# ml-jku/LaM-SLidE

Measured on AMD Instinct MI355X. Metric: sampled trajectories/sec (50-step ODE) + decoded-coord L2 vs ref, MD17, higher is better.
Workload: dtype bf16; 1 GPU; md17_bench; tail=False, ln_fuse=True, T=30, L=256, C=32, D=512, H=16, depth=4, sampler=ODE, state_updates=50, batch_per_gpu=32, global_batch=32, parallelism=batch-shard x1, 1 gather to rank 0 per step, noise_elem_stride_per_rank=7864320, kernels=general, trajectories_per_pass=32

## Files before the change

### lam_slide_amd/csrc/k_lin1.hip.h

```cpp
#pragma once
#include <type_traits>

#include "common.hip.h"

struct Lin1Args {
    const u16 *W;
    const u16 *X;
    const float *bias;
    const float4 *rope_q, *rope_k;
    u16 *qkv;
    u16 *z;
    int F, N, HHD, M;
    int pos_div, pos_mod;
    unsigned div_magic, mod_magic;
    float inv_hd, q_premul;
    int nt;
    int wpt;
    int planes;
    int npad;
    const float2 *ln_stat;
    const float *ln_shift, *ln_scale;
    int ln_mod_stride, ln_tpt;
    unsigned ln_tpt_magic;
};

#ifndef LIN1_B2
#define LIN1_B2 1
#endif
#ifndef LIN1_B2_KMAX
#define LIN1_B2_KMAX 256
#endif

template <int HDP, int K, int NW = 8>
struct Lin1Cfg {
    static_assert(K % 128 == 0 && K <= 512, "hidden sizes 128 / 256 / 384 / 512");
    static constexpr int KS = K / 16;
    static constexpr int ROWB = 2 * K;
    static constexpr int PITCH = ROWB + 16;
    static constexpr int BLK = 32 * PITCH;
    static constexpr int NS = (LIN1_B2 && K <= LIN1_B2_KMAX) ? 4 : 3;
    static constexpr int RING = NS * BLK;
    static_assert(NW == 8 || NW == 4, "two waves per SIMD (256-token tiles) or one (128-token tiles)");
    static constexpr int TT = 32 * NW;
    static constexpr int STAGE = NW * 4096;
    static constexpr int LPR = ROWB / 16;
    static constexpr int PPW = 32 / NW;
    static constexpr size_t lds_bytes(int F) { return (size_t)RING + STAGE + (size_t)F * 4; }
    static constexpr int LN_SLOTS = K <= 256 ? 3 : 2;
    static constexpr size_t lds_bytes_lnf(int F) { return lds_bytes(F) + (size_t)LN_SLOTS * 2 * K * 4; }
};

enum { LIN1_QK = 0, LIN1_V = 1, LIN1_MLP = 2 };

#ifndef LIN1_XLOAD
#define LIN1_XLOAD 1
#endif
#ifndef LIN1_PD
#define LIN1_PD 3
#endif

__device__ __forceinline__ float lin1_gelu(float x) {
    const float ax = fabsf(x);
    const float h = __builtin_amdgcn_exp2f(LSL_GELU_Q(ax));
    float relu;
    asm("v_max_f32 %0, 0, %1" : "=v"(relu) : "v"(x));
    return fmaf(-ax, h, relu);
}

template <int HDP, int K, int NW = 8, bool LNF = false>
__global__ void __launch_bounds__(NW * 64, NW / 4) k_linear1_ts(Lin1Args g) {
    using C = Lin1Cfg<HDP, K, NW>;
    constexpr int KS = C::KS, BLK = C::BLK, PPW = C::PPW, ROWB = C::ROWB;
    constexpr int NCO = HDP == 32 ? 8 : 4;
    extern __shared__ __attribute__((aligned(16))) char smem[];

    const int tid = threadIdx.x, lane = tid & 63;
    const int wave = __builtin_amdgcn_readfirstlane(tid >> 6);
    const int r = lane & 31, hf = lane >> 5;
    char *const stage = smem + C::RING + wave * 4096;
    float *const bias_lds = reinterpret_cast<float *>(smem + C::RING + C::STAGE);

    const int NB = g.F >> 5;
    const int ntile = (g.N + C::TT - 1) / C::TT;
    const long U = (long)ntile * NB;
    long i0, i1;
    if (g.wpt > 0) {
        const int tile = blockIdx.x / g.wpt, part = blockIdx.x - tile * g.wpt;
        i0 = (long)tile * NB + ((NB * part / g.wpt) & ~1);
        i1 = (long)tile * NB + (part + 1 == g.wpt ? NB : ((NB * (part + 1) / g.wpt) & ~1));
    } else {
        i0 = (U * blockIdx.x / gridDim.x) & ~1L;
        i1 = blockIdx.x + 1 == gridDim.x ? U : ((U * (blockIdx.x + 1) / gridDim.x) & ~1L);
    }
    if (i0 >= i1) return;

    for (int i = tid * 4; i < g.F; i += NW * 64 * 4) *reinterpret_cast<float4 *>(bias_lds + i) = *reinterpret_cast<const float4 *>(g.bias + i);

    const unsigned lds0 = (unsigned)(size_t)(LDS_PTR(char))(smem);
    const unsigned lane_src = lane * 16;
    const char *const w_rows = reinterpret_cast<const char *>(g.W) + (size_t)(PPW * wave) * ROWB;
    auto issue_piece = [&](const char *src, unsigned dst, auto ic) __attribute__((always_inline)) {
        constexpr int I = decltype(ic)::value & 3;
        if (decltype(ic)::value >= 4) {
            src += 4 * ROWB;
            dst += 4 * C::PITCH;
        }
        const unsigned ls = lane_src;
        if (C::LPR == 64 || lane < C::LPR) {
            if (I == 0 || decltype(ic)::value >= 4)
                asm volatile("s_add_u32 m0, %2, %3\n\ts_nop 4\n\tglobal_load_lds_dwordx4 %0, %1 offset:%4" ::"v"(ls), "s"(src), "s"(dst), "n"(16 * I), "n"(ROWB * I) : "memory", "scc");
            else
                asm volatile("s_add_u32 m0, %2, %3\n\ts_nop 0\n\tglobal_load_lds_dwordx4 %0, %1 offset:%4" ::"v"(ls), "s"(src), "s"(dst), "n"(16 * I), "n"(ROWB * I) : "memory", "scc");
        }
    };
    auto req_src = [&](int blk) __attribute__((always_inline)) { return w_rows + (size_t)blk * (32 * ROWB); };
    auto req_dst = [&](int slot) __attribute__((always_inline)) { return lds0 + slot * BLK + PPW * wave * C::PITCH; };
    auto issue = [&](int blk, int slot) __attribute__((always_inline)) {
        const char *src = req_src(blk);
        const unsigned dst = req_dst(slot);
        issue_piece(src, dst, std::integral_constant<int, 0>());
        issue_piece(src, dst, std::integral_constant<int, 1>());
        issue_piece(src, dst, std::integral_constant<int, 2>());
        issue_piece(src, dst, std::integral_constant<int, 3>());
        if (PPW == 8) {
            issue_piece(src, dst, std::integral_constant<int, 4>());
            issue_piece(src, dst, std::integral_constant<int, 5>());
            issue_piece(src, dst, std::integral_constant<int, 6>());
            issue_piece(src, dst, std::integral_constant<int, 7>());
        }
    };
    const int aoff = r * C::PITCH + 16 * hf;

    bf16x8 xreg[KS];
    float4 co[NCO];
    f32x16 acc0, acc1;
    int slot_c = 0;
    int dma_blk, dma_slot;
    int n_wave = 0;
    float post = 1.0f;

    auto advance = [&](int &b) __attribute__((always_inline)) { b = b + 1 == NB ? 0 : b + 1; };
    auto next_slot = [&](int s) __attribute__((always_inline)) { return s == C::NS - 1 ? 0 : s + 1; };

    {
        int b = (int)(i0 - (i0 / NB) * NB);
        issue(b, 0);
        advance(b);
        issue(b, 1);
        advance(b);
        dma_blk = b;
        dma_slot = 2;
    }

    auto init_acc = [&](f32x16 &a, int blk) __attribute__((always_inline)) {
#pragma unroll
        for (int q4 = 0; q4 < 4; ++q4) {
            const float4 b = *reinterpret_cast<const float4 *>(bias_lds + blk * 32 + 8 * q4 + 4 * hf);
            a[4 * q4] = b.x; a[4 * q4 + 1] = b.y; a[4 * q4 + 2] = b.z; a[4 * q4 + 3] = b.w;
        }
    };
    constexpr bool B2 = LIN1_B2 != 0 && K <= LIN1_B2_KMAX;
    auto step_head = [&](auto flushed_c) __attribute__((always_inline)) {
        if (B2) {
            if (decltype(flushed_c)::value) wait_vmcnt<PPW>();
            else wait_vmcnt<0>();
        } else {
            if (decltype(flushed_c)::value) wait_vmcnt<2 * PPW>();
            else wait_vmcnt<PPW>();
        }
        __builtin_amdgcn_s_barrier();
        asm volatile("" ::: "memory");
    };
    const unsigned wr0 = (unsigned)(size_t)(LDS_PTR(char))(stage) + r * 128 + 8 * hf + ((r & 7) << 4);
    const unsigned rd0 = (unsigned)(size_t)(LDS_PTR(char))(stage) + (lane >> 3) * 128 + (((lane & 7) ^ ((lane >> 3) & 7)) << 4);
    const char *row_q = nullptr, *row_z = nullptr;
    const bool planes = g.planes != 0;
    constexpr unsigned PROW = 2u * HDP, CPH = HDP / 8;
    const unsigned plane_bytes = PROW * (unsigned)g.npad;
    const unsigned stride_q = planes ? PROW : 2u * 3 * g.HHD, stride_z = 2u * (g.HHD + g.M);
    const unsigned blk_q = planes ? (32 / HDP) * plane_bytes : 64u;
    const unsigned voff_q = planes ? ((lane & 7) / CPH) * plane_bytes + (lane >> 3) * PROW + 16 * ((lane & 7) % CPH) : (lane >> 3) * stride_q + 16 * (lane & 7);
    const unsigned voff_z = (lane >> 3) * stride_z + 16 * (lane & 7);
    const int slab_z = 3 * (g.HHD >> 5);
    const char *fl_base = nullptr;
    unsigned fl_stride8 = 0, fl_voff = 0;
    auto flush_setup = [&](int b_even) __attribute__((always_inline)) {
        const bool to_qkv = b_even < slab_z;
        fl_base = to_qkv ? row_q : row_z;
        fl_stride8 = 8 * (to_qkv ? stride_q : stride_z);
        fl_voff = to_qkv ? voff_q + blk_q * (unsigned)b_even : voff_z + 64u * (unsigned)b_even;
    };
    auto flush_read = [&](int half, u32x4 (&pk)[2]) __attribute__((always_inline)) {
#pragma unroll
        for (int i = 0; i < 2; ++i) pk[i] = *reinterpret_cast<const LDS_PTR(u32x4)>(rd0 + 1024 * (2 * half + i));
    };
    auto flush_store = [&](int half, const u32x4 (&pk)[2]) __attribute__((always_inline)) {
        asm volatile("s_nop 4\n\tglobal_store_dwordx4 %0, %1, %2 nt\n\ts_nop 1" ::"v"(fl_voff + (2 * half) * fl_stride8), "v"(pk[0]), "s"(fl_base) : "memory");
        asm volatile("global_store_dwordx4 %0, %1, %2 nt\n\ts_nop 1" ::"v"(fl_voff + (2 * half + 1) * fl_stride8), "v"(pk[1]), "s"(fl_base) : "memory");
    };
    auto flush_store_visible = [&](int half, const u32x4 (&pk)[2]) __attribute__((always_inline)) {
#pragma unroll
        for (int i = 0; i < 2; ++i)
            __builtin_nontemporal_store(pk[i], reinterpret_cast<u32x4 *>(const_cast<char *>(fl_base) + (size_t)(fl_voff + (2 * half + i) * fl_stride8)));
    };
    auto put_group = [&](int ii, int q, float v0, float v1, float v2, float v3) __attribute__((always_inline)) {
        const u32x2 pk = {pack2(v0, v1), pack2(v2, v3)};
        *reinterpret_cast<LDS_PTR(u32x2)>(wr0 ^ (unsigned)(64 * ii + 16 * q)) = pk;
    };
    auto epi_slice = [&](auto sec_c, int s, const f32x16 &a, int ii, float &c0, float &c1) __attribute__((always_inline)) {
        constexpr int SEC = decltype(sec_c)::value;
        if constexpr (SEC == LIN1_QK && HDP == 32) {
            if (s == 0) c0 = 0.0f;
            if (s < 2) {
#pragma unroll
                for (int e = 0; e < 8; ++e) c0 = fmaf(a[8 * s + e], a[8 * s + e], c0);
            }
            if (s == 1) c0 = rsqrtf(fmaf(half_pair_sum(c0), g.inv_hd, 1e-6f)) * post;
            if (s >= 2 && s < 6) {
                const int q = s - 2;
                float o[4];
#pragma unroll
                for (int kk = 0; kk < 2; ++kk) {
                    const int k = 2 * q + kk;
                    const float x0 = a[2 * k], x1 = a[2 * k + 1];
                    o[2 * kk] = c0 * fmaf(co[k].x, x0, -co[k].y * x1);
                    o[2 * kk + 1] = c0 * fmaf(co[k].z, x0, co[k].w * x1);
                }
                put_group(ii, q, o[0], o[1], o[2], o[3]);
            }
        } else if constexpr (SEC == LIN1_QK) {
            if (s == 0) {
                c0 = 0.0f;
#pragma unroll
                for (int e = 0; e < 8; ++e) c0 = fmaf(a[e], a[e], c0);
            }
            if (s == 1) {
                c1 = 0.0f;
#pragma unroll
                for (int e = 0; e < 8; ++e) c1 = fmaf(a[8 + e], a[8 + e], c1);
                c0 = rsqrtf(fmaf(half_pair_sum(c0), g.inv_hd, 1e-6f)) * post;
                c1 = rsqrtf(fmaf(half_pair_sum(c1), g.inv_hd, 1e-6f)) * post;
            }
            if (s >= 2 && s < 6) {
                const int q = s - 2;
                const float rr = q < 2 ? c0 : c1;
                float o[4];
#pragma unroll
                for (int kk = 0; kk < 2; ++kk) {
                    const int k = 2 * q + kk;
                    const float x0 = a[2 * k], x1 = a[2 * k + 1];
                    const float4 cf = co[k & (NCO - 1)];
                    o[2 * kk] = rr * fmaf(cf.x, x0, -cf.y * x1);
                    o[2 * kk + 1] = rr * fmaf(cf.z, x0, cf.w * x1);
                }
                put_group(ii, q, o[0], o[1], o[2], o[3]);
            }
        } else if constexpr (SEC == LIN1_MLP) {
            const float g0 = lin1_gelu(a[2 * s]), g1 = lin1_gelu(a[2 * s + 1]);
            if (s & 1) put_group(ii, s >> 1, c0, c1, g0, g1);
            else { c0 = g0; c1 = g1; }
        } else {
            if (s < 4) put_group(ii, s, a[4 * s], a[4 * s + 1], a[4 * s + 2], a[4 * s + 3]);
        }
    };
    auto step = [&](auto sec_c, auto par_c, auto mfma_c, auto epi_c, auto side) __attribute__((always_inline)) {
        constexpr int PAR = decltype(par_c)::value;
        constexpr bool DO_MFMA = decltype(mfma_c)::value != 0, DO_EPI = decltype(epi_c)::value != 0;
        constexpr int MPS = KS / 8, PD = LIN1_PD, MH = (MPS + 1) / 2;
        f32x16 &ac = PAR ? acc0 : acc1;
        const f32x16 &ae = PAR ? acc1 : acc0;
        const char *sb = smem + slot_c * BLK + aoff;
        bf16x8 fr[PD];
        float c0 = 0.0f, c1 = 0.0f;
        if (DO_MFMA) {
#pragma unroll
            for (int ks = 0; ks < PD; ++ks) fr[ks] = as_bf16x8(*reinterpret_cast<const u32x4 *>(sb + 32 * ks));
        }
        side(std::integral_constant<int, -1>());
#define LIN1_SIDE(S) if (s == S) side(std::integral_constant<int, S>());
#pragma unroll
        for (int s = 0; s < 8; ++s) {
#pragma unroll
            for (int m = 0; m < MPS; ++m) {
                if (m == MH) { LIN1_SIDE(0) LIN1_SIDE(1) LIN1_SIDE(2) LIN1_SIDE(3) LIN1_SIDE(4) LIN1_SIDE(5) LIN1_SIDE(6) LIN1_SIDE(7) }
                if (DO_MFMA) {
                    const int ks = s * MPS + m;
                    ac = mfma32(fr[ks % PD], xreg[ks], ac);
                    if (ks + PD < KS) fr[ks % PD] = as_bf16x8(*reinterpret_cast<const u32x4 *>(sb + 32 * (ks + PD)));
                }
            }
            if (MH == MPS) { LIN1_SIDE(0) LIN1_SIDE(1) LIN1_SIDE(2) LIN1_SIDE(3) LIN1_SIDE(4) LIN1_SIDE(5) LIN1_SIDE(6) LIN1_SIDE(7) }
            if (DO_EPI) epi_slice(sec_c, s, ae, PAR, c0, c1);
            __builtin_amdgcn_sched_barrier(0);
        }
#undef LIN1_SIDE
        if (decltype(mfma_c)::value != 0) slot_c = next_slot(slot_c);
    };
    std::integral_constant<int, 0> I0;
    std::integral_constant<int, 1> I1;
    auto no_side = [](auto) __attribute__((always_inline)) {};
    auto fused = [&](auto sec_c, auto par_c, auto flush_c, auto prev_c, int e) __attribute__((always_inline)) {
        constexpr int PAR = decltype(par_c)::value;
        constexpr bool FLUSH = decltype(flush_c)::value != 0;
        if (!B2 || PAR == 1) step_head(prev_c);
        u32x4 pk[2];
        if (FLUSH) flush_setup(e - 2);
        const char *src = req_src(dma_blk);
        const unsigned dst = req_dst(dma_slot);
        int blk2 = dma_blk;
        advance(blk2);
        const char *src2 = req_src(blk2);
        const unsigned dst2 = req_dst(next_slot(dma_slot));
        init_acc(PAR ? acc0 : acc1, e + 1);
        step(sec_c, par_c, I1, I1, [&](auto sl) __attribute__((always_inline)) {
            constexpr int SL = decltype(sl)::value;
            if (FLUSH) {
                if (SL == -1) flush_read(0, pk);
                if (SL == 0) {
                    flush_store(0, pk);
                    flush_read(1, pk);
                }
                if (SL == 1) flush_store(1, pk);
            }
            constexpr int PS = PPW / 4;
            if (!B2) {
                if (SL >= 2 && SL < 6) {
                    issue_piece(src, dst, std::integral_constant<int, (SL >= 2 && SL < 6) ? PS * (SL - 2) : 0>());
                    if (PS == 2) issue_piece(src, dst, std::integral_constant<int, (SL >= 2 && SL < 6) ? PS * (SL - 2) + 1 : 0>());
                }
            } else if (PAR == 1) {
                if (SL >= 0 && SL < 4) {
                    issue_piece(src, dst, std::integral_constant<int, (SL >= 0 && SL < 4) ? PS * SL : 0>());
                    if (PS == 2) issue_piece(src, dst, std::integral_constant<int, (SL >= 0 && SL < 4) ? PS * SL + 1 : 0>());
                }
                if (SL >= 4 && SL < 8) {
                    issue_piece(src2, dst2, std::integral_constant<int, (SL >= 4 && SL < 8) ? PS * (SL - 4) : 0>());
                    if (PS == 2) issue_piece(src2, dst2, std::integral_constant<int, (SL >= 4 && SL < 8) ? PS * (SL - 4) + 1 : 0>());
                }
            }
        });
        if (!B2) {
            advance(dma_blk);
            dma_slot = next_slot(dma_slot);
        } else if (PAR == 1) {
            advance(dma_blk);
            advance(dma_blk);
            dma_slot = next_slot(next_slot(dma_slot));
        }
    };
    auto run = [&](auto sec_c, int ea, int eb) __attribute__((always_inline)) {
        int e = ea;
        if (e < eb && (e & 1)) {
            fused(sec_c, I1, I0, I0, e);
            ++e;
        }
        for (; e + 1 < eb; e += 2) {
            fused(sec_c, I0, I1, I0, e);
            fused(sec_c, I1, I0, I1, e + 1);
        }
        if (e < eb) fused(sec_c, I0, I1, I0, e);
    };
    auto load_co = [&](const float4 *tab, unsigned pos) __attribute__((always_inline)) {
        const float4 *t = tab + (size_t)pos * (HDP / 2) + 2 * hf;
#pragma unroll
        for (int k = 0; k < NCO; ++k) co[k] = t[4 * (k >> 1) + (k & 1)];
    };
    std::integral_constant<int, LIN1_QK> SQK;
    std::integral_constant<int, LIN1_V> SV;
    std::integral_constant<int, LIN1_MLP> SMLP;

    constexpr bool XLINES = LIN1_XLOAD != 0 && (K <= 384 || LIN1_XLOAD >= 2);
    auto load_x = [&](int nw) __attribute__((always_inline)) {
        if (!XLINES) {
            const u16 *xr = g.X + (size_t)(nw + r) * K + 8 * hf;
#pragma unroll
            for (int ks = 0; ks < KS; ++ks) xreg[ks] = as_bf16x8(*reinterpret_cast<const u32x4 *>(xr + 16 * ks));
        } else {
            const u16 *xr = g.X + (size_t)(nw + (lane >> 3)) * K + 8 * (lane & 7);
#pragma unroll
            for (int j = 0; j < KS / 4; ++j)
#pragma unroll
                for (int q = 0; q < 4; ++q) xreg[4 * j + q] = as_bf16x8(*reinterpret_cast<const u32x4 *>(xr + (size_t)(8 * q) * K + 64 * j));
        }
    };
    auto finish_x = [&]() __attribute__((always_inline)) {
        if (!XLINES) return;
        const unsigned t0 = lane >> 3;
        const unsigned xw = (unsigned)(size_t)(LDS_PTR(char))(stage) + t0 * 128;
        const unsigned xr0 = (unsigned)(size_t)(LDS_PTR(char))(stage) + r * 128;
#pragma unroll
        for (int j = 0; j < KS / 4; ++j) {
#pragma unroll
            for (int q = 0; q < 4; ++q)
                *reinterpret_cast<LDS_PTR(u32x4)>(xw + 1024 * q + ((((lane & 7) ^ ((t0 >> 1) + 4 * q)) & 7) << 4)) = as_u32x4(xreg[4 * j + q]);
#pragma unroll
            for (int m = 0; m < 4; ++m)
                xreg[4 * j + m] = as_bf16x8(*reinterpret_cast<const LDS_PTR(u32x4)>(xr0 + ((((2 * m + hf) ^ (r >> 1)) & 7) << 4)));
        }
    };

    float *const ln_tab = bias_lds + ((g.F + 3) & ~3);
    auto traj_of = [&](unsigned n) __attribute__((always_inline)) { return g.ln_tpt_magic ? __umulhi(n, g.ln_tpt_magic) : n; };
    auto load_x_lnf = [&](int tile_, int nw) __attribute__((always_inline)) {
        typedef __attribute__((ext_vector_type(4))) float f4;
        const float *xf = reinterpret_cast<const float *>(g.X);
        const unsigned t_first = g.ln_mod_stride ? traj_of((unsigned)(tile_ * C::TT)) : 0u;
        const unsigned t_last = g.ln_mod_stride ? traj_of((unsigned)(g.N - 1)) : 0u;
        for (int i = tid * 4; i < C::LN_SLOTS * K; i += NW * 64 * 4) {
            const int slot = i / K, col = i - slot * K;
            const size_t mo = (size_t)min(t_first + (unsigned)slot, t_last) * g.ln_mod_stride + col;
            const f4 sc = *reinterpret_cast<const f4 *>(g.ln_scale + mo), sh = *reinterpret_cast<const f4 *>(g.ln_shift + mo);
            *reinterpret_cast<f4 *>(ln_tab + (size_t)slot * 2 * K + col) = f4{1.0f + sc[0], 1.0f + sc[1], 1.0f + sc[2], 1.0f + sc[3]};
            *reinterpret_cast<f4 *>(ln_tab + (size_t)slot * 2 * K + K + col) = sh;
        }
        const unsigned rowi = lane >> 3, chunk = lane & 7;
        const unsigned sbase = (unsigned)(size_t)(LDS_PTR(char))(stage);
        const unsigned xr0 = sbase + r * 128;
        const float *xr = xf + (size_t)(nw + rowi) * K + 4 * chunk;
        float2 st[4];
        const float *tb[4];
#pragma unroll
        for (int q = 0; q < 4; ++q) {
            const unsigned nn = (unsigned)min(nw + (int)rowi + 8 * q, g.N - 1);
            st[q] = g.ln_stat[nn];
            const unsigned slot = g.ln_mod_stride ? min(traj_of(nn) - t_first, (unsigned)(C::LN_SLOTS - 1)) : 0u;
            tb[q] = ln_tab + (size_t)slot * 2 * K + 4 * chunk;
        }
        __syncthreads();
#pragma unroll
        for (int p = 0; p < K / 64; ++p) {
            f4 v[2][4];
#pragma unroll
            for (int e = 0; e < 2; ++e)
#pragma unroll
                for (int q = 0; q < 4; ++q) v[e][q] = *reinterpret_cast<const f4 *>(xr + (size_t)(8 * q) * K + 64 * p + 32 * e);
#pragma unroll
            for (int q = 0; q < 4; ++q) {
                const unsigned row = rowi + 8 * q, sw = (row >> 1) & 7;
#pragma unroll
                for (int e = 0; e < 2; ++e) {
                    const f4 sc = *reinterpret_cast<const f4 *>(tb[q] + 64 * p + 32 * e), sh = *reinterpret_cast<const f4 *>(tb[q] + K + 64 * p + 32 * e);
                    f4 x = v[e][q];
#pragma unroll
                    for (int c = 0; c < 4; ++c) x[c] = fmaf(x[c], st[q].x, st[q].y) * sc[c] + sh[c];
                    const u32x2 pk = {pack2(x[0], x[1]), pack2(x[2], x[3])};
                    *reinterpret_cast<LDS_PTR(u32x2)>(sbase + row * 128 + ((((4 * e + (chunk >> 1)) ^ sw) & 7) << 4) + 8 * (chunk & 1)) = pk;
                }
            }
#pragma unroll
            for (int m = 0; m < 4; ++m)
                xreg[4 * p + m] = as_bf16x8(*reinterpret_cast<const LDS_PTR(u32x4)>(xr0 + ((((2 * m + hf) ^ (r >> 1)) & 7) << 4)));
            __builtin_amdgcn_sched_barrier(0);
        }
    };
    const int qb = g.HHD >> 5;
    int tile = (int)(i0 / NB), b0 = (int)(i0 - (long)tile * NB), left = (int)(i1 - i0);
    bool first_seg = true;
    bool co_ready = false;
    __syncthreads();
    while (left > 0) {
        const int b1 = NB - b0 < left ? NB : b0 + left;
        n_wave = tile * C::TT + wave * 32;
        row_q = reinterpret_cast<const char *>(g.qkv) + (size_t)n_wave * stride_q;
        row_z = reinterpret_cast<const char *>(g.z) + (size_t)n_wave * stride_z - 4 * (size_t)g.HHD;
        if constexpr (LNF) load_x_lnf(tile, n_wave);
        else {
            if (first_seg) load_x(n_wave);
            finish_x();
        }
        const unsigned nn = (unsigned)min(n_wave + r, g.N - 1);
        const unsigned n1 = g.div_magic ? __umulhi(nn, g.div_magic) : nn;
        const unsigned pos = g.mod_magic ? n1 - __umulhi(n1, g.mod_magic) * (unsigned)g.pos_mod : 0u;

        if (first_seg) wait_vmcnt<0>();
        else wait_vmcnt<4>();
        __builtin_amdgcn_s_barrier();
        asm volatile("" ::: "memory");
        issue(dma_blk, dma_slot);
        advance(dma_blk);
        dma_slot = next_slot(dma_slot);
        if (B2) {
            issue(dma_blk, dma_slot);
            advance(dma_blk);
            dma_slot = next_slot(dma_slot);
        }
        init_acc(acc0, b0);
        step(SV, I1, I1, I0, no_side);
        const int e_end = b1 - 1;
        if (b0 < 2 * qb) {
            if (!co_ready) load_co(b0 < qb ? g.rope_q : g.rope_k, pos);
            post = b0 < qb ? g.q_premul : 1.0f;
            fused(SQK, I0, I0, I0, b0);
        } else if (b0 < 3 * qb) {
            fused(SV, I0, I0, I0, b0);
        } else {
            fused(SMLP, I0, I0, I0, b0);
        }
        {
            const int lo = max(b0 + 1, 0), hi = min(e_end, qb);
            if (lo < hi) run(SQK, lo, hi);
        }
        {
            const int lo = max(b0 + 1, qb), hi = min(e_end, 2 * qb);
            if (lo < hi) {
                if (lo == qb) {
                    load_co(g.rope_k, pos);
                    post = 1.0f;
                }
                run(SQK, lo, hi);
            }
        }
        {
            const int lo = max(b0 + 1, 2 * qb), hi = min(e_end, 3 * qb);
            if (lo < hi) run(SV, lo, hi);
        }
        {
            const int lo = max(b0 + 1, 3 * qb), hi = min(e_end, NB);
            if (lo < hi) run(SMLP, lo, hi);
        }
        const int left_next = left - (b1 - b0);
        co_ready = false;
        if (left_next > 0) {
            asm volatile("" ::: "memory");
            const int nw = (tile + 1) * C::TT + wave * 32;
            if constexpr (!LNF) load_x(nw);
            if (b1 - 1 >= 2 * qb) {
                const unsigned nn2 = (unsigned)min(nw + r, g.N - 1);
                const unsigned m1 = g.div_magic ? __umulhi(nn2, g.div_magic) : nn2;
                load_co(g.rope_q, g.mod_magic ? m1 - __umulhi(m1, g.mod_magic) * (unsigned)g.pos_mod : 0u);
                co_ready = true;
            }
            asm volatile("" ::: "memory");
        }
        {
            const int e = b1 - 1;
            if (e < 2 * qb) {
                step(SQK, I1, I0, I1, no_side);
            } else if (e < 3 * qb) {
                step(SV, I1, I0, I1, no_side);
            } else {
                step(SMLP, I1, I0, I1, no_side);
            }
            flush_setup(e - 1);
            u32x4 pk[2];
            flush_read(0, pk);
            flush_store_visible(0, pk);
            flush_read(1, pk);
            flush_store_visible(1, pk);
        }
        left = left_next;
        tile += 1;
        b0 = 0;
        first_seg = false;
    }
    wait_vmcnt<0>();
}
```

### lam_slide_amd/csrc/k_lin2.hip.h

```cpp
#pragma once
#include <type_traits>

#include "common.hip.h"

struct Lin2Args {
    const u16 *Wp;
    const u16 *Z;
    const float *bias;
    const float *gate;
    float *h;
    int F, N;
    int mod_stride, tpt;
    unsigned tpt_magic;
    int slices, rpx;
    int gate_rows;
    float2 *stats;
    int npad;
};

#ifndef LIN2_PD
#define LIN2_PD 2
#endif

template <int N, int I = 0, class F>
__device__ __forceinline__ void static_for(F &f) {
    if constexpr (I < N) {
        f(std::integral_constant<int, I>());
        static_for<N, I + 1>(f);
    }
}

template <int K, int NCH, int NS, bool HB2>
struct Lin2Cfg {
    static_assert(K % (32 * NCH) == 0, "K / 2 splits into NCH chunks of whole 16-deep k-steps");
    static_assert(NCH >= 3 && NS >= 3, "epilogue schedule: arithmetic, stores, residual request in chunks 0, 1, 2");
    static constexpr int KH = K / 2;
    static constexpr int KSH = KH / 16;
    static constexpr int KC = KH / NCH;
    static constexpr int MPC = KC / 16;
    static constexpr int ROWB = 4 * KC;
    static constexpr int LPR = ROWB / 16;
    static_assert(LPR <= 64, "one DMA instruction per token row");
    static constexpr int PITCH = ROWB + 16;
    static constexpr int CHUNK = 32 * PITCH;
    static constexpr int RING = NS * CHUNK;
    static constexpr int EXCH = RING;
    static constexpr int HBUF = EXCH + 4 * 4096;
    static constexpr int HB_PER_WAVE = HB2 ? 8192 : 4096;
    static constexpr int BIAS = HBUF + 4 * HB_PER_WAVE;
    static constexpr int GATE = BIAS + 512;
    static constexpr size_t lds_bytes(int gate_rows) { return (size_t)GATE + (size_t)gate_rows * 512; }
    static constexpr int max_gate_rows = (163840 - GATE) / 512;
    static_assert(max_gate_rows >= 1, "LDS budget (160 KiB per workgroup)");
};

__global__ void __launch_bounds__(256) k_lin2_pack(u16 *out, const u16 *W, int F, int K) {
    const int ksh = K / 32;
    const long total = (long)(F / 32) * 2 * ksh * 64;
    for (long i = (long)blockIdx.x * 256 + threadIdx.x; i < total; i += (long)gridDim.x * 256) {
        const int lane = (int)(i & 63);
        long t = i >> 6;
        const int ks = (int)(t % ksh);
        t /= ksh;
        const int o = (int)(t & 1), fb = (int)(t >> 1);
        const u16 *src = W + (size_t)(32 * fb + (lane & 31)) * K + o * (K / 2) + 16 * ks + 8 * (lane >> 5);
        *reinterpret_cast<u32x4 *>(out + i * 8) = *reinterpret_cast<const u32x4 *>(src);
    }
}

template <int K, int NCH, int NS, bool HB2, bool LNS = false>
__global__ void __launch_bounds__(512, 2) k_linear2_ws(Lin2Args g) {
    using C = Lin2Cfg<K, NCH, NS, HB2>;
    constexpr int KSH = C::KSH, KC = C::KC, MPC = C::MPC, PITCH = C::PITCH, CHUNK = C::CHUNK, PD = LIN2_PD;
    extern __shared__ __attribute__((aligned(16))) char smem[];

    const int tid = threadIdx.x, lane = tid & 63;
    const int wave = __builtin_amdgcn_readfirstlane(tid >> 6);
    const int r = lane & 31, hf = lane >> 5;
    const int hi = wave >> 2;
    const int p = wave & 3;

    const int xcd = blockIdx.x & 7, idx = blockIdx.x >> 3;
    const int slice = idx % g.slices, range = xcd * g.rpx + idx / g.slices, ranges = 8 * g.rpx;
    const int NBLK = (g.N + 31) >> 5;
    const int blk0 = (int)((long)NBLK * range / ranges), blk1 = (int)((long)NBLK * (range + 1) / ranges);
    const int nblk = blk1 - blk0;
    if (nblk <= 0) return;
    const int f0 = slice * 128 + 32 * p;

    const unsigned lds0 = (unsigned)(size_t)(LDS_PTR(char))(smem);
    float *const bias_lds = reinterpret_cast<float *>(smem + C::BIAS);
    float *const gate_lds = reinterpret_cast<float *>(smem + C::GATE);

    bf16x8 wreg[KSH];
    {
        const u32x4 *wp = reinterpret_cast<const u32x4 *>(g.Wp) + ((size_t)((slice * 4 + p) * 2 + hi) * KSH) * 64 + lane;
#pragma unroll
        for (int ks = 0; ks < KSH; ++ks) wreg[ks] = as_bf16x8(wp[(size_t)ks * 64]);
    }
    const int n_lo = blk0 * 32, n_hi = min(blk1 * 32, g.N) - 1;
    const unsigned traj_lo = g.mod_stride ? (g.tpt_magic ? __umulhi((unsigned)n_lo, g.tpt_magic) : (unsigned)n_lo) : 0u;
    {
        const unsigned traj_hi = g.mod_stride ? (g.tpt_magic ? __umulhi((unsigned)n_hi, g.tpt_magic) : (unsigned)n_hi) : 0u;
        const int rows = min((int)(traj_hi - traj_lo) + 1, g.gate_rows);
        if (tid < 32) *reinterpret_cast<float4 *>(bias_lds + 4 * tid) = *reinterpret_cast<const float4 *>(g.bias + slice * 128 + 4 * tid);
        for (int i = tid; i < rows * 32; i += 512) {
            const int row = i >> 5, c4 = i & 31;
            *reinterpret_cast<float4 *>(gate_lds + row * 128 + 4 * c4) =
                *reinterpret_cast<const float4 *>(g.gate + (size_t)(traj_lo + row) * g.mod_stride + slice * 128 + 4 * c4);
        }
    }

    const unsigned half_lanes = C::LPR / 2;
    const unsigned voff_same = lane < half_lanes ? 16u * lane : (unsigned)K + 16u * (lane - half_lanes);
    const unsigned voff_next = lane < half_lanes ? 64u * K + 16u * lane : (unsigned)K + 16u * (lane - half_lanes);
    auto dma_row = [&](const char *src_, unsigned dst_, unsigned voff) __attribute__((always_inline)) {
        const char *src = uni_ptr(src_);
        const unsigned dst = __builtin_amdgcn_readfirstlane(dst_);
        if (C::LPR == 64 || lane < C::LPR) lds_dma16(voff, src, dst);
    };
    auto chunk_src = [&](int m, int j, unsigned &voff) __attribute__((always_inline)) {
        int mh = min(max(m - 1, 0), nblk - 1), ml = min(m, nblk - 1);
        voff = ml > mh ? voff_next : voff_same;
        return reinterpret_cast<const char *>(g.Z) + ((size_t)(blk0 + mh) * 32 + 8 * p) * (2 * K) + (size_t)j * (2 * KC);
    };

    const int boff = r * PITCH + (hi * KC + 8 * hf) * 2;
    f32x16 acc;
#pragma unroll
    for (int e = 0; e < 16; ++e) acc[e] = 0.0f;

    auto chain = [&](auto jc, int slot, bool zero_start, auto side) __attribute__((always_inline)) {
        constexpr int J = decltype(jc)::value;
        const char *sb = smem + slot * CHUNK + boff;
        bf16x8 fr[PD];
#pragma unroll
        for (int i = 0; i < PD; ++i) fr[i] = as_bf16x8(*reinterpret_cast<const u32x4 *>(sb + 32 * i));
#pragma unroll
        for (int i = 0; i < MPC; ++i) {
            if (J == 0 && i == 0 && zero_start) {
                f32x16 z;
#pragma unroll
                for (int e = 0; e < 16; ++e) z[e] = 0.0f;
                acc = mfma32(wreg[J * MPC + i], fr[i % PD], z);
            } else
                acc = mfma32(wreg[J * MPC + i], fr[i % PD], acc);
            if (i + PD < MPC) fr[i % PD] = as_bf16x8(*reinterpret_cast<const u32x4 *>(sb + 32 * (i + PD)));
            side(i);
            __builtin_amdgcn_sched_barrier(0);
        }
    };
    char *const exch = smem + C::EXCH + p * 4096;
    auto next_slot = [](int s) __attribute__((always_inline)) { return s + 1 == NS ? 0 : s + 1; };

    __builtin_amdgcn_s_waitcnt(0x0F70);
    __syncthreads();

    if (!hi) {
        int rq_m = 0, rq_j = 0, rq_slot = 0;
        auto rq_advance = [&]() __attribute__((always_inline)) {
            if (++rq_j == NCH) { rq_j = 0; ++rq_m; }
            rq_slot = next_slot(rq_slot);
        };
#pragma unroll
        for (int c = 0; c < NS - 1; ++c) {
            unsigned voff;
            const char *src = chunk_src(rq_m, rq_j, voff);
            const unsigned dst = lds0 + rq_slot * CHUNK + 8 * p * PITCH;
#pragma unroll
            for (int i = 0; i < 8; ++i) dma_row(src + (size_t)i * (2 * K), dst + i * PITCH, voff);
            rq_advance();
        }
        int slot = 0;
        for (int m = 0; m <= nblk; ++m) {
            const bool work = m < nblk;
            auto step = [&](auto jc) __attribute__((always_inline)) {
                wait_vmcnt<8 * (NS - 2)>();
                __builtin_amdgcn_s_barrier();
                asm volatile("" ::: "memory");
                unsigned voff;
                const char *src = chunk_src(rq_m, rq_j, voff);
                const unsigned dst = lds0 + rq_slot * CHUNK + 8 * p * PITCH;
                rq_advance();
                if (work) {
                    chain(jc, slot, true, [&](int i) __attribute__((always_inline)) {
                        if (i % 2 == 1 && i / 2 < 8) dma_row(src + (size_t)(i / 2) * (2 * K), dst + (i / 2) * PITCH, voff);
                    });
                    if (MPC < 16) {
#pragma unroll
                        for (int i = MPC / 2; i < 8; ++i) dma_row(src + (size_t)i * (2 * K), dst + i * PITCH, voff);
                    }
                } else {
#pragma unroll
                    for (int i = 0; i < 8; ++i) dma_row(src + (size_t)i * (2 * K), dst + i * PITCH, voff);
                }
                slot = next_slot(slot);
            };
            static_for<NCH>(step);
            if (work) {
#pragma unroll
                for (int q = 0; q < 4; ++q)
                    *reinterpret_cast<float4 *>(exch + q * 1024 + lane * 16) = make_float4(acc[4 * q], acc[4 * q + 1], acc[4 * q + 2], acc[4 * q + 3]);
                asm volatile("s_waitcnt lgkmcnt(0)" ::: "memory");
            }
        }
        wait_vmcnt<0>();
        return;
    }

    char *const hbuf = smem + C::HBUF + p * C::HB_PER_WAVE;
    const unsigned hbuf_lds = lds0 + C::HBUF + p * C::HB_PER_WAVE;
    const unsigned row_bytes = 4u * g.F;
    auto hb_off = [](int b) __attribute__((always_inline)) { return HB2 ? (b & 1) * 4096 : 0; };
    auto opaque_lane = [&]() __attribute__((always_inline)) {
        int l = lane;
        asm volatile("" : "+v"(l));
        return l;
    };
    auto h_request = [&](int b) __attribute__((always_inline)) {
        const int l = opaque_lane(), tr = l >> 3, ch = (l & 7) ^ (tr & 7);
#pragma unroll
        for (int i = 0; i < 4; ++i) {
            const unsigned n = (unsigned)min((blk0 + b) * 32 + 8 * i + tr, g.N - 1);
            const unsigned voff = n * row_bytes + 4u * f0 + 16u * ch, dst = __builtin_amdgcn_readfirstlane(hbuf_lds + hb_off(b) + i * 1024);
            lds_dma16(voff, g.h, dst);
        }
    };
    auto epi_stats_regs = [&](int b, const float4 (&w)[4]) __attribute__((always_inline)) {
        const int l = opaque_lane(), rr = l & 31, hh = l >> 5;
        const int n_row = (blk0 + b) * 32 + rr;
        float s1 = 0.0f;
#pragma unroll
        for (int q = 0; q < 4; ++q) s1 += (w[q].x + w[q].y) + (w[q].z + w[q].w);
        const float m16 = s1 * (1.0f / 16.0f);
        float q16 = 0.0f;
#pragma unroll
        for (int q = 0; q < 4; ++q) {
            const float dx = w[q].x - m16, dy = w[q].y - m16, dz = w[q].z - m16, dw = w[q].w - m16;
            q16 += (dx * dx + dy * dy) + (dz * dz + dw * dw);
        }
        const auto pm = __builtin_amdgcn_permlane32_swap(__float_as_uint(m16), __float_as_uint(m16), false, false);
        const auto pq = __builtin_amdgcn_permlane32_swap(__float_as_uint(q16), __float_as_uint(q16), false, false);
        const float m_lo = __uint_as_float((unsigned)pm[0]), m_hi = __uint_as_float((unsigned)pm[1]), dm = m_lo - m_hi;
        const u32x2 st = {__float_as_uint(0.5f * (m_lo + m_hi)),
                          __float_as_uint((__uint_as_float((unsigned)pq[0]) + __uint_as_float((unsigned)pq[1])) + 8.0f * dm * dm)};
        if (hh == 0 && n_row < g.N) {
            const unsigned voff = (unsigned)(((f0 >> 5) * g.npad + n_row) * 8);
            asm volatile("s_nop 4\n\tglobal_store_dwordx2 %0, %1, %2\n\ts_nop 1" ::"v"(voff), "v"(st), "s"(g.stats) : "memory");
        }
    };
    auto epi_math = [&](int b) __attribute__((always_inline)) {
        const int l = opaque_lane(), rr = l & 31, hh = l >> 5;
        const int n_row = (blk0 + b) * 32 + rr;
        const unsigned n = (unsigned)min(n_row, g.N - 1);
        const unsigned traj = g.mod_stride ? (g.tpt_magic ? __umulhi(n, g.tpt_magic) : n) - traj_lo : 0u;
        const float *bp = bias_lds + 32 * p + 4 * hh, *gp = gate_lds + traj * 128 + 32 * p + 4 * hh;
        char *hrow = hbuf + hb_off(b) + rr * 128;
        float4 w[4];
#pragma unroll
        for (int q = 0; q < 4; ++q) {
            const float4 bs = *reinterpret_cast<const float4 *>(bp + 8 * q);
            const float4 gt = *reinterpret_cast<const float4 *>(gp + 8 * q);
            float4 *hp = reinterpret_cast<float4 *>(hrow + 16 * ((2 * q + hh) ^ (rr & 7)));
            float4 hv = *hp;
            hv.x = fmaf(gt.x, acc[4 * q] + bs.x, hv.x);
            hv.y = fmaf(gt.y, acc[4 * q + 1] + bs.y, hv.y);
            hv.z = fmaf(gt.z, acc[4 * q + 2] + bs.z, hv.z);
            hv.w = fmaf(gt.w, acc[4 * q + 3] + bs.w, hv.w);
            *hp = hv;
            if constexpr (LNS) w[q] = hv;
        }
        if constexpr (LNS) epi_stats_regs(b, w);
    };
    auto epi_store = [&](int b, int i, bool ragged) __attribute__((always_inline)) {
        const int l = opaque_lane(), tr = l >> 3, ch = (l & 7) ^ (tr & 7);
        const u32x4 v = *reinterpret_cast<const u32x4 *>(hbuf + hb_off(b) + i * 1024 + l * 16);
        const int n = (blk0 + b) * 32 + 8 * i + tr;
        const unsigned voff = (unsigned)min(n, g.N - 1) * row_bytes + 4u * f0 + 16u * ch;
        if (ragged) {
            if (n < g.N) store16(reinterpret_cast<char *>(g.h) + voff, v, true);
        } else
            asm volatile("s_nop 4\n\tglobal_store_dwordx4 %0, %1, %2 nt\n\ts_nop 1" ::"v"(voff), "v"(v), "s"(g.h) : "memory");
    };

    int slot = 0;
    if (HB2) h_request(0);
    for (int c = 0; c < NCH; ++c) {
        __builtin_amdgcn_s_barrier();
        slot = next_slot(slot);
    }
    for (int m = 1; m <= nblk; ++m) {
        const int B = m - 1;
        auto step = [&](auto jc) __attribute__((always_inline)) {
            constexpr int J = decltype(jc)::value;
            __builtin_amdgcn_s_barrier();
            asm volatile("" ::: "memory");
            if (J == 0) {
                if (B >= 1) {
                    if (!HB2) wait_vmcnt<0>();
                    else if (B >= 2) wait_vmcnt<8 + (LNS ? 1 : 0)>();
                    else wait_vmcnt<4>();
                    asm volatile("" ::: "memory");
                    epi_math(B - 1);
                }
                const int l = opaque_lane();
#pragma unroll
                for (int q = 0; q < 4; ++q) {
                    const float4 v = *reinterpret_cast<const float4 *>(exch + q * 1024 + l * 16);
                    acc[4 * q] = v.x; acc[4 * q + 1] = v.y; acc[4 * q + 2] = v.z; acc[4 * q + 3] = v.w;
                }
            }
            constexpr int GAP = MPC >= 13 ? 3 : MPC >= 9 ? 2 : 1, IN_CHAIN = (MPC - 2) / GAP + 1 < 4 ? (MPC - 2) / GAP + 1 : 4;
            chain(jc, slot, false, [&](int i) __attribute__((always_inline)) {
                if (J == 1 && B >= 1 && i >= 1 && (i - 1) % GAP == 0 && (i - 1) / GAP < IN_CHAIN) epi_store(B - 1, (i - 1) / GAP, false);
                if (J == 2 && i == 1) h_request(HB2 ? min(B + 1, nblk - 1) : B);
            });
            if (J == 1 && B >= 1) {
#pragma unroll
                for (int k = IN_CHAIN; k < 4; ++k) epi_store(B - 1, k, false);
            }
            slot = next_slot(slot);
        };
        static_for<NCH>(step);
    }
    wait_vmcnt<0>();
    asm volatile("" ::: "memory");
    {
        const int b = nblk - 1;
        const bool ragged = (blk0 + b) * 32 + 32 > g.N;
        epi_math(b);
#pragma unroll
        for (int i = 0; i < 4; ++i) epi_store(b, i, ragged);
    }
    wait_vmcnt<0>();
}
```

Baseline: 57.51 trajectories/s.

## Prefetch next tile's LN-fused X rows during drain and pair LN-stat stores

In the LN-fused linear1 kernel, the next tile's X rows, LN stats and modulation table are now requested before the current tile's drain and flush, and consumed afterward. A configurable prefetch depth is added, and the flush stores are interleaved into the LN finish so that the global-load latency hides behind the drain. In linear2, LN statistics from even blocks are held in registers and written together with odd blocks using both half-waves, which halves the number of store instructions. Both changes retune vmcnt waits, which adds register pressure and makes the wait counts fragile.

```diff
diff --git a/lam_slide_amd/csrc/k_lin1.hip.h b/lam_slide_amd/csrc/k_lin1.hip.h
--- a/lam_slide_amd/csrc/k_lin1.hip.h
+++ b/lam_slide_amd/csrc/k_lin1.hip.h
@@ -55,6 +55,9 @@
 #ifndef LIN1_XLOAD
 #define LIN1_XLOAD 1
 #endif
+#ifndef LIN1_LNF_DEPTH
+#define LIN1_LNF_DEPTH 1
+#endif
 #ifndef LIN1_PD
 #define LIN1_PD 3
 #endif
@@ -138,6 +141,7 @@
     int dma_blk, dma_slot;
     int n_wave = 0;
     float post = 1.0f;
+    bool first_seg = true;
 
     auto advance = [&](int &b) __attribute__((always_inline)) { b = b + 1 == NB ? 0 : b + 1; };
     auto next_slot = [&](int s) __attribute__((always_inline)) { return s == C::NS - 1 ? 0 : s + 1; };
@@ -162,10 +166,13 @@
     constexpr bool B2 = LIN1_B2 != 0 && K <= LIN1_B2_KMAX;
     auto step_head = [&](auto flushed_c) __attribute__((always_inline)) {
         if (B2) {
-            if (decltype(flushed_c)::value) wait_vmcnt<PPW>();
+            if (decltype(flushed_c)::value == 1) wait_vmcnt<PPW>();
             else wait_vmcnt<0>();
+        } else if (LNF && decltype(flushed_c)::value == 2) {
+            if (first_seg) wait_vmcnt<PPW>();
+            else wait_vmcnt<4 + NCO + PPW>();
         } else {
-            if (decltype(flushed_c)::value) wait_vmcnt<2 * PPW>();
+            if (decltype(flushed_c)::value == 1) wait_vmcnt<2 * PPW>();
             else wait_vmcnt<PPW>();
         }
         __builtin_amdgcn_s_barrier();
@@ -298,6 +305,7 @@
     };
     std::integral_constant<int, 0> I0;
     std::integral_constant<int, 1> I1;
+    std::integral_constant<int, 2> I2;
     auto no_side = [](auto) __attribute__((always_inline)) {};
     auto fused = [&](auto sec_c, auto par_c, auto flush_c, auto prev_c, int e) __attribute__((always_inline)) {
         constexpr int PAR = decltype(par_c)::value;
@@ -400,71 +408,120 @@
     };
 
     float *const ln_tab = bias_lds + ((g.F + 3) & ~3);
+    typedef __attribute__((ext_vector_type(4))) float lnf4;
+    constexpr int LNF_NP = K / 64, LNF_DEPTH = LNF_NP < LIN1_LNF_DEPTH ? LNF_NP : LIN1_LNF_DEPTH, LNF_NBUF = LNF_DEPTH + 1;
+    static_assert(C::LN_SLOTS * K <= NW * 64 * 4, "one table element group per thread");
+    struct LnfRows {
+        lnf4 v[LNF_NBUF][2][4];
+        float2 st[4];
+        lnf4 tab[2];
+    };
     auto traj_of = [&](unsigned n) __attribute__((always_inline)) { return g.ln_tpt_magic ? __umulhi(n, g.ln_tpt_magic) : n; };
-    auto load_x_lnf = [&](int tile_, int nw) __attribute__((always_inline)) {
-        typedef __attribute__((ext_vector_type(4))) float f4;
-        const float *xf = reinterpret_cast<const float *>(g.X);
+    auto lnf_tab_store = [&](lnf4 sc, lnf4 sh) __attribute__((always_inline)) {
+        const int i = tid * 4, slot = i / K, col = i - slot * K;
+        if (i < C::LN_SLOTS * K) {
+            *reinterpret_cast<lnf4 *>(ln_tab + (size_t)slot * 2 * K + col) = lnf4{1.0f + sc[0], 1.0f + sc[1], 1.0f + sc[2], 1.0f + sc[3]};
+            *reinterpret_cast<lnf4 *>(ln_tab + (size_t)slot * 2 * K + K + col) = sh;
+        }
+    };
+    auto lnf_tab_load = [&](LnfRows &L, int tile_) __attribute__((always_inline)) {
         const unsigned t_first = g.ln_mod_stride ? traj_of((unsigned)(tile_ * C::TT)) : 0u;
         const unsigned t_last = g.ln_mod_stride ? traj_of((unsigned)(g.N - 1)) : 0u;
-        for (int i = tid * 4; i < C::LN_SLOTS * K; i += NW * 64 * 4) {
-            const int slot = i / K, col = i - slot * K;
-            const size_t mo = (size_t)min(t_first + (unsigned)slot, t_last) * g.ln_mod_stride + col;
-            const f4 sc = *reinterpret_cast<const f4 *>(g.ln_scale + mo), sh = *reinterpret_cast<const f4 *>(g.ln_shift + mo);
-            *reinterpret_cast<f4 *>(ln_tab + (size_t)slot * 2 * K + col) = f4{1.0f + sc[0], 1.0f + sc[1], 1.0f + sc[2], 1.0f + sc[3]};
-            *reinterpret_cast<f4 *>(ln_tab + (size_t)slot * 2 * K + K + col) = sh;
-        }
-        const unsigned rowi = lane >> 3, chunk = lane & 7;
+        const int i = min(tid * 4, C::LN_SLOTS * K - 4), slot = i / K, col = i - slot * K;
+        const size_t mo = (size_t)min(t_first + (unsigned)slot, t_last) * g.ln_mod_stride + col;
+        L.tab[0] = *reinterpret_cast<const lnf4 *>(g.ln_scale + mo);
+        L.tab[1] = *reinterpret_cast<const lnf4 *>(g.ln_shift + mo);
+    };
+    auto lnf_lane = [&]() __attribute__((always_inline)) {
+        int l = lane;
+        asm volatile("" : "+v"(l));
+        return l;
+    };
+    auto lnf_rows = [&](int nw, int l) __attribute__((always_inline)) {
+        return reinterpret_cast<const float *>(g.X) + (size_t)(nw + (l >> 3)) * K + 4 * (l & 7);
+    };
+    auto lnf_issue = [&](LnfRows &L, const float *xr, int P) __attribute__((always_inline)) {
+#pragma unroll
+        for (int e = 0; e < 2; ++e)
+#pragma unroll
+            for (int q = 0; q < 4; ++q) L.v[P % LNF_NBUF][e][q] = *reinterpret_cast<const lnf4 *>(xr + (size_t)(8 * q) * K + 64 * P + 32 * e);
+    };
+    auto lnf_request = [&](LnfRows &L, int tile_, int nw) __attribute__((always_inline)) {
+        const int l = lnf_lane();
+        const float *xr = lnf_rows(nw, l);
+#pragma unroll
+        for (int q = 0; q < 4; ++q) L.st[q] = g.ln_stat[min(nw + (l >> 3) + 8 * q, g.N - 1)];
+        if (g.ln_mod_stride) lnf_tab_load(L, tile_);
+#pragma unroll
+        for (int p = 0; p < LNF_DEPTH; ++p) lnf_issue(L, xr, p);
+    };
+    auto lnf_finish = [&](LnfRows &L, int tile_, int nw, auto slab_stores) __attribute__((always_inline)) {
+        const int l = lnf_lane();
+        const unsigned rowi = l >> 3, chunk = l & 7, r_ = l & 31, hf_ = l >> 5;
         const unsigned sbase = (unsigned)(size_t)(LDS_PTR(char))(stage);
-        const unsigned xr0 = sbase + r * 128;
-        const float *xr = xf + (size_t)(nw + rowi) * K + 4 * chunk;
-        float2 st[4];
-        const float *tb[4];
+        const unsigned xr0 = sbase + r_ * 128;
+        const float *xr = lnf_rows(nw, l);
+        const unsigned t_first = g.ln_mod_stride ? traj_of((unsigned)(tile_ * C::TT)) : 0u;
+        if (g.ln_mod_stride) {
+            lnf_tab_store(L.tab[0], L.tab[1]);
+            __syncthreads();
+        }
+        unsigned tb[4];
 #pragma unroll
         for (int q = 0; q < 4; ++q) {
             const unsigned nn = (unsigned)min(nw + (int)rowi + 8 * q, g.N - 1);
-            st[q] = g.ln_stat[nn];
             const unsigned slot = g.ln_mod_stride ? min(traj_of(nn) - t_first, (unsigned)(C::LN_SLOTS - 1)) : 0u;
-            tb[q] = ln_tab + (size_t)slot * 2 * K + 4 * chunk;
-        }
-        __syncthreads();
-#pragma unroll
-        for (int p = 0; p < K / 64; ++p) {
-            f4 v[2][4];
-#pragma unroll
-            for (int e = 0; e < 2; ++e)
-#pragma unroll
-                for (int q = 0; q < 4; ++q) v[e][q] = *reinterpret_cast<const f4 *>(xr + (size_t)(8 * q) * K + 64 * p + 32 * e);
+            tb[q] = (unsigned)(size_t)(LDS_PTR(char))(reinterpret_cast<char *>(ln_tab)) + (slot * 2 * K + 4 * chunk) * 4;
+        }
+        if (LNF_NP == LNF_DEPTH) slab_stores();
+#pragma unroll
+        for (int p = 0; p < LNF_NP; ++p) {
+            if (p + LNF_DEPTH < LNF_NP) {
+                lnf_issue(L, xr, p + LNF_DEPTH);
+                if (p + LNF_DEPTH == LNF_NP - 1) slab_stores();
+                __builtin_amdgcn_sched_barrier(0);
+            }
 #pragma unroll
             for (int q = 0; q < 4; ++q) {
                 const unsigned row = rowi + 8 * q, sw = (row >> 1) & 7;
 #pragma unroll
                 for (int e = 0; e < 2; ++e) {
-                    const f4 sc = *reinterpret_cast<const f4 *>(tb[q] + 64 * p + 32 * e), sh = *reinterpret_cast<const f4 *>(tb[q] + K + 64 * p + 32 * e);
-                    f4 x = v[e][q];
-#pragma unroll
-                    for (int c = 0; c < 4; ++c) x[c] = fmaf(x[c], st[q].x, st[q].y) * sc[c] + sh[c];
+                    const lnf4 sc = *reinterpret_cast<const LDS_PTR(lnf4)>(tb[q] + 4 * (64 * p + 32 * e)), sh = *reinterpret_cast<const LDS_PTR(lnf4)>(tb[q] + 4 * (K + 64 * p + 32 * e));
+                    lnf4 x = L.v[p % LNF_NBUF][e][q];
+#pragma unroll
+                    for (int c = 0; c < 4; ++c) x[c] = fmaf(x[c], L.st[q].x, L.st[q].y) * sc[c] + sh[c];
                     const u32x2 pk = {pack2(x[0], x[1]), pack2(x[2], x[3])};
                     *reinterpret_cast<LDS_PTR(u32x2)>(sbase + row * 128 + ((((4 * e + (chunk >> 1)) ^ sw) & 7) << 4) + 8 * (chunk & 1)) = pk;
                 }
             }
 #pragma unroll
             for (int m = 0; m < 4; ++m)
-                xreg[4 * p + m] = as_bf16x8(*reinterpret_cast<const LDS_PTR(u32x4)>(xr0 + ((((2 * m + hf) ^ (r >> 1)) & 7) << 4)));
+                xreg[4 * p + m] = as_bf16x8(*reinterpret_cast<const LDS_PTR(u32x4)>(xr0 + ((((2 * m + hf_) ^ (r_ >> 1)) & 7) << 4)));
             __builtin_amdgcn_sched_barrier(0);
         }
     };
     const int qb = g.HHD >> 5;
     int tile = (int)(i0 / NB), b0 = (int)(i0 - (long)tile * NB), left = (int)(i1 - i0);
-    bool first_seg = true;
     bool co_ready = false;
-    __syncthreads();
+    if constexpr (LNF) {
+        const int nw = tile * C::TT + wave * 32;
+        LnfRows L;
+        lnf_request(L, tile, nw);
+        if (!g.ln_mod_stride) {
+            LnfRows T;
+            lnf_tab_load(T, 0);
+            lnf_tab_store(T.tab[0], T.tab[1]);
+        }
+        __syncthreads();
+        lnf_finish(L, tile, nw, []() __attribute__((always_inline)) {});
+    } else
+        __syncthreads();
     while (left > 0) {
         const int b1 = NB - b0 < left ? NB : b0 + left;
         n_wave = tile * C::TT + wave * 32;
         row_q = reinterpret_cast<const char *>(g.qkv) + (size_t)n_wave * stride_q;
         row_z = reinterpret_cast<const char *>(g.z) + (size_t)n_wave * stride_z - 4 * (size_t)g.HHD;
-        if constexpr (LNF) load_x_lnf(tile, n_wave);
-        else {
+        if constexpr (!LNF) {
             if (first_seg) load_x(n_wave);
             finish_x();
         }
@@ -473,7 +530,7 @@
         const unsigned pos = g.mod_magic ? n1 - __umulhi(n1, g.mod_magic) * (unsigned)g.pos_mod : 0u;
 
         if (first_seg) wait_vmcnt<0>();
-        else wait_vmcnt<4>();
+        else wait_vmcnt<LNF ? 4 + NCO : 4>();
         __builtin_amdgcn_s_barrier();
         asm volatile("" ::: "memory");
         issue(dma_blk, dma_slot);
@@ -490,11 +547,11 @@
         if (b0 < 2 * qb) {
             if (!co_ready) load_co(b0 < qb ? g.rope_q : g.rope_k, pos);
             post = b0 < qb ? g.q_premul : 1.0f;
-            fused(SQK, I0, I0, I0, b0);
+            fused(SQK, I0, I0, I2, b0);
         } else if (b0 < 3 * qb) {
-            fused(SV, I0, I0, I0, b0);
+            fused(SV, I0, I0, I2, b0);
         } else {
-            fused(SMLP, I0, I0, I0, b0);
+            fused(SMLP, I0, I0, I2, b0);
         }
         {
             const int lo = max(b0 + 1, 0), hi = min(e_end, qb);
@@ -520,19 +577,15 @@
         }
         const int left_next = left - (b1 - b0);
         co_ready = false;
-        if (left_next > 0) {
-            asm volatile("" ::: "memory");
-            const int nw = (tile + 1) * C::TT + wave * 32;
-            if constexpr (!LNF) load_x(nw);
-            if (b1 - 1 >= 2 * qb) {
+        auto next_co = [&](int nw, auto always_c) __attribute__((always_inline)) {
+            if (decltype(always_c)::value || b1 - 1 >= 2 * qb) {
                 const unsigned nn2 = (unsigned)min(nw + r, g.N - 1);
                 const unsigned m1 = g.div_magic ? __umulhi(nn2, g.div_magic) : nn2;
                 load_co(g.rope_q, g.mod_magic ? m1 - __umulhi(m1, g.mod_magic) * (unsigned)g.pos_mod : 0u);
                 co_ready = true;
             }
-            asm volatile("" ::: "memory");
-        }
-        {
+        };
+        auto drain = [&]() __attribute__((always_inline)) {
             const int e = b1 - 1;
             if (e < 2 * qb) {
                 step(SQK, I1, I0, I1, no_side);
@@ -542,6 +595,39 @@
                 step(SMLP, I1, I0, I1, no_side);
             }
             flush_setup(e - 1);
+        };
+        if constexpr (LNF) {
+            u32x4 pk[2], pk1[2];
+            if (left_next <= 0) {
+                drain();
+                flush_read(0, pk);
+                flush_store_visible(0, pk);
+                flush_read(1, pk);
+                flush_store_visible(1, pk);
+                break;
+            }
+            LnfRows L;
+            const int nw = (tile + 1) * C::TT + wave * 32;
+            asm volatile("" ::: "memory");
+            lnf_request(L, tile + 1, nw);
+            asm volatile("" ::: "memory");
+            drain();
+            flush_read(0, pk);
+            flush_read(1, pk1);
+            lnf_finish(L, tile + 1, nw, [&]() __attribute__((always_inline)) {
+                flush_store_visible(0, pk);
+                flush_store_visible(1, pk1);
+            });
+            next_co(nw, I1);
+        } else {
+            if (left_next > 0) {
+                asm volatile("" ::: "memory");
+                const int nw = (tile + 1) * C::TT + wave * 32;
+                load_x(nw);
+                next_co(nw, I0);
+                asm volatile("" ::: "memory");
+            }
+            drain();
             u32x4 pk[2];
             flush_read(0, pk);
             flush_store_visible(0, pk);
diff --git a/lam_slide_amd/csrc/k_lin2.hip.h b/lam_slide_amd/csrc/k_lin2.hip.h
--- a/lam_slide_amd/csrc/k_lin2.hip.h
+++ b/lam_slide_amd/csrc/k_lin2.hip.h
@@ -226,9 +226,9 @@
             lds_dma16(voff, g.h, dst);
         }
     };
+    u32x2 st_even = {0u, 0u};
     auto epi_stats_regs = [&](int b, const float4 (&w)[4]) __attribute__((always_inline)) {
         const int l = opaque_lane(), rr = l & 31, hh = l >> 5;
-        const int n_row = (blk0 + b) * 32 + rr;
         float s1 = 0.0f;
 #pragma unroll
         for (int q = 0; q < 4; ++q) s1 += (w[q].x + w[q].y) + (w[q].z + w[q].w);
@@ -244,10 +244,21 @@
         const float m_lo = __uint_as_float((unsigned)pm[0]), m_hi = __uint_as_float((unsigned)pm[1]), dm = m_lo - m_hi;
         const u32x2 st = {__float_as_uint(0.5f * (m_lo + m_hi)),
                           __float_as_uint((__uint_as_float((unsigned)pq[0]) + __uint_as_float((unsigned)pq[1])) + 8.0f * dm * dm)};
-        if (hh == 0 && n_row < g.N) {
-            const unsigned voff = (unsigned)(((f0 >> 5) * g.npad + n_row) * 8);
-            asm volatile("s_nop 4\n\tglobal_store_dwordx2 %0, %1, %2\n\ts_nop 1" ::"v"(voff), "v"(st), "s"(g.stats) : "memory");
-        }
+        if (b & 1) {
+            const int n_row = (blk0 + b - 1 + hh) * 32 + rr;
+            const u32x2 sv = {hh ? st[0] : st_even[0], hh ? st[1] : st_even[1]};
+            if (n_row < g.N) {
+                const unsigned voff = (unsigned)(((f0 >> 5) * g.npad + n_row) * 8);
+                asm volatile("s_nop 4\n\tglobal_store_dwordx2 %0, %1, %2\n\ts_nop 1" ::"v"(voff), "v"(sv), "s"(g.stats) : "memory");
+            }
+        } else if (b == nblk - 1) {
+            const int n_row = (blk0 + b) * 32 + rr;
+            if (hh == 0 && n_row < g.N) {
+                const unsigned voff = (unsigned)(((f0 >> 5) * g.npad + n_row) * 8);
+                asm volatile("s_nop 4\n\tglobal_store_dwordx2 %0, %1, %2\n\ts_nop 1" ::"v"(voff), "v"(st), "s"(g.stats) : "memory");
+            }
+        } else
+            st_even = st;
     };
     auto epi_math = [&](int b) __attribute__((always_inline)) {
         const int l = opaque_lane(), rr = l & 31, hh = l >> 5;
@@ -298,7 +309,10 @@
             if (J == 0) {
                 if (B >= 1) {
                     if (!HB2) wait_vmcnt<0>();
-                    else if (B >= 2) wait_vmcnt<8 + (LNS ? 1 : 0)>();
+                    else if (B >= 2) {
+                        if (LNS && (B & 1)) wait_vmcnt<9>();
+                        else wait_vmcnt<8>();
+                    }
                     else wait_vmcnt<4>();
                     asm volatile("" ::: "memory");
                     epi_math(B - 1);
```

Result: no change. 57.24 trajectories/s (-0.5%).
